# liamhebert/MultiModalDiscussionTransformer

Measured on AMD Instinct MI355X. Metric: discussion-tree comments/sec fwd+bwd, higher is better.
Workload: dtype bf16; 1 GPU; mDT-base (BERT-base + ViT-B/16 split 6+6, 6 executed graph layers, D768 H12 nb4 L100), 32 bushy 64-comment trees per GPU, 25% image comments, random-init weights, dropout 0.4/0.3/0.3 (run_train.sh:37), token lengths U{8..100} zero-padded to 100 (SURVEY.md §8d; mean 54.3 valid tokens), text side ragged: padded token positions are not computed (identical logits / gradients), last fusion layer comput; trees_per_gpu=32, parallelism=dp1, frozen_initial_encoders=False

## Files before the change

### multimodaldiscussiontransformer_amd/csrc/gemm.hip

```cpp
#include <stdlib.h>

#include <algorithm>
#include <type_traits>
#include <vector>

#include "common.hpp"
#include "gemm_tiles.hpp"
#include "gemm_epilogue.hpp"

namespace mdt {

template <typename TIn, typename TOut, bool TA, bool TB>
__global__ __launch_bounds__(256) void gemm_generic_kernel(GemmParams p) {
  constexpr int BM = 64, BN = 64, BK = 16, LD = 68;
  __shared__ float As[BK][LD];
  __shared__ float Bs[BK][LD];
  const int tid = threadIdx.x, lane = tid & 63, wave = tid >> 6;
  const int wr = wave >> 1, wc = wave & 1;
  const int64_t m0 = (int64_t)blockIdx.y * BM, n0 = (int64_t)blockIdx.x * BN;
  const int64_t kbeg = (int64_t)blockIdx.z * p.k_chunk;
  const int64_t kend = (kbeg + p.k_chunk < p.K) ? kbeg + p.k_chunk : p.K;
  const TIn* A = (const TIn*)p.A;
  const TIn* B = (const TIn*)p.B;
  f32x4 acc[2][2];
// ... 894 lines not shown
  }
  __shared__ float red[4][64 * VN];
#pragma unroll
  for (int e = 0; e < VN; ++e) red[wave][lane * VN + e] = acc[e];
  __syncthreads();
  for (int i = threadIdx.x; i < 64 * VN; i += 256) {
    const int64_t col = (int64_t)blockIdx.x * 64 * VN + i;
    if (col < N) atomicAdd(out + col, red[0][i] + red[1][i] + red[2][i] + red[3][i]);
  }
}

template <typename T>
__global__ __launch_bounds__(256) void dropout_kernel(int64_t rows, int D, const T* x, int64_t ldx, T* y, int64_t ldy, DropCfg d) {
  const int lane = threadIdx.x & 63;
  for (int64_t r = (int64_t)blockIdx.x * 4 + (threadIdx.x >> 6); r < rows; r += (int64_t)gridDim.x * 4)
    for (int c = lane; c < D; c += 64)
      y[r * ldy + c] = from_f32<T>(to_f32(x[r * ldx + c]) * drop_scale(d, (uint64_t)r * D + c));
}
template <typename T, int VN>
__global__ __launch_bounds__(256) void dropout_vec_kernel(int64_t rows, int D, const T* x, int64_t ldx, T* y, int64_t ldy, DropCfg d) {
  typedef __attribute__((ext_vector_type(VN))) T vec;
  const int lane = threadIdx.x & 63;
  for (int64_t r = (int64_t)blockIdx.x * 4 + (threadIdx.x >> 6); r < rows; r += (int64_t)gridDim.x * 4)
    for (int c = lane * VN; c < D; c += 64 * VN) {
      const vec v = *(const vec*)(x + r * ldx + c);
      vec o;
#pragma unroll
      for (int e = 0; e < VN; e += 2) {
        float s0, s1;
        drop_scale2(d, (uint64_t)r * D + c + e, s0, s1);
        o[e] = from_f32<T>(to_f32((T)v[e]) * s0);
        o[e + 1] = from_f32<T>(to_f32((T)v[e + 1]) * s1);
      }
      *(vec*)(y + r * ldy + c) = o;
    }
}
__global__ void dropout_mask_kernel(int64_t n, DropCfg d, uint8_t* mask) {
  for (int64_t i = (int64_t)blockIdx.x * blockDim.x + threadIdx.x; i < n; i += (int64_t)gridDim.x * blockDim.x)
    mask[i] = drop_scale(d, (uint64_t)i) != 0.f;
}

template <typename TS, typename TD>
__global__ void cast_kernel(int64_t n, const TS* s, TD* d) {
  for (int64_t i = (int64_t)blockIdx.x * blockDim.x + threadIdx.x; i < n; i += (int64_t)gridDim.x * blockDim.x)
    d[i] = from_f32<TD>(to_f32(s[i]));
}

template <typename TS, typename TD>
__global__ __launch_bounds__(256) void transpose_kernel(int64_t rows, int64_t cols, const TS* s, int64_t lds_, TD* d,
                                                        int64_t ldd) {
  __shared__ float tile[32][33];
  const int64_t r0 = (int64_t)blockIdx.y * 32, c0 = (int64_t)blockIdx.x * 32;
  const int tx = threadIdx.x & 31, ty = threadIdx.x >> 5;
  for (int i = ty; i < 32; i += 8)
    if (r0 + i < rows && c0 + tx < cols) tile[i][tx] = to_f32(s[(r0 + i) * lds_ + c0 + tx]);
  __syncthreads();
  for (int i = ty; i < 32; i += 8)
    if (c0 + i < cols && r0 + tx < rows) d[(c0 + i) * ldd + r0 + tx] = from_f32<TD>(tile[tx][i]);
}

static void report_stamps(unsigned long long* dev, size_t nwg, const GemmParams& p) {
  std::vector<unsigned long long> h(nwg * 4);
  if (hipDeviceSynchronize() != hipSuccess || hipMemcpy(h.data(), dev, nwg * 32, hipMemcpyDeviceToHost) != hipSuccess) { (void)hipGetLastError(); return; }
  std::vector<double> cyc, clk;
  unsigned long long t0 = ~0ull, t1 = 0;
  for (size_t i = 0; i < nwg; ++i) {
    if (h[4 * i + 2] == 0 || h[4 * i + 1] == 0) continue;
    cyc.push_back((double)h[4 * i] / (double)h[4 * i + 2]);
    clk.push_back((double)h[4 * i] / (double)h[4 * i + 1] * 100.0);
    t0 = std::min(t0, h[4 * i + 3]);
    t1 = std::max(t1, h[4 * i + 3] + h[4 * i + 1]);
  }
  if (cyc.empty()) return;
  std::sort(cyc.begin(), cyc.end());
  std::sort(clk.begin(), clk.end());
  fprintf(stderr, "[mdt gemm stamp] M=%lld N=%lld K=%lld wgs=%zu  cycles/k-tile median %.0f (p10 %.0f p90 %.0f)  clock median %.0f MHz  span %.1f us\n",
          (long long)p.M, (long long)p.N, (long long)p.K, nwg, cyc[cyc.size() / 2], cyc[cyc.size() / 10], cyc[cyc.size() * 9 / 10],
          clk[clk.size() / 2], (double)(t1 - t0) / 100.0);
  std::vector<unsigned long long> st(256);
  if (hipMemcpy(st.data(), dev + nwg * 4, 256 * 8, hipMemcpyDeviceToHost) == hipSuccess && st[0]) {
    fprintf(stderr, "[mdt gemm steps]");
    for (int i = 1; i < 256 && st[i]; ++i) fprintf(stderr, " %llu", st[i] - st[i - 1]);
    fprintf(stderr, "\n");
  } else (void)hipGetLastError();
}

static int num_cus() {
  const int n = device_cus() & ~7;
  return n < 8 ? 8 : n;
}

static int* g_tile_queues = nullptr;
static int g_tile_queue_sets = 0;

static int xcd_group_n(int tiles_m, int tiles_n, double b_panel, int n_cus) {
  if (tiles_n % 2 == 0 && b_panel * tiles_n > 3.5e6 && b_panel * (tiles_n / 2) <= 2.5e6 && (double)tiles_m * tiles_n >= 4.0 * n_cus)
    return tiles_n / 2;
  return tiles_n;
}

struct GemmPlan {
  GemmRoute route;
  int tiles_m, tiles_n, split_k, group_n;
  int64_t k_chunk;
  dim3 grid;
  bool strip_asum;
};

static GemmPlan plan_gemm(const GemmParams& p, int dtype, int out_dtype, int ta, int tb, int n_cus) {
  const Switches& sw = switches();
  const int64_t M = p.M, N = p.N, K = p.K;
  const int epi = p.epilogue;
  bool fast = dtype == MDT_BF16 && K > 0 && (ta ? M % T_BM == 0 : K % T_BK == 0) && (tb ? N % T_BN == 0 : K % T_BK == 0) &&
              N % T_BN == 0 && p.lda % 8 == 0 && p.ldb % 8 == 0 && ((uintptr_t)p.A | (uintptr_t)p.B) % 16 == 0 &&
              p.lda * 2 * 128 < (1ll << 31) && p.ldb * 2 * 128 < (1ll << 31);
  const int ov = out_dtype == MDT_F32 ? 4 : 8;
  if (!(epi & MDT_EPI_ATOMIC) && (p.ldc % ov || ((uintptr_t)p.C & 15))) fast = false;
  if ((epi & MDT_EPI_BIAS) && ((uintptr_t)p.bias & 15)) fast = false;
  if ((epi & MDT_EPI_RESIDUAL) && (p.ldr % 8 || ((uintptr_t)p.residual & 15))) fast = false;
  if (p.aux && (p.ldaux % 8 || ((uintptr_t)p.aux & 15))) fast = false;
  const int64_t chunk = ((K + p.split_k - 1) / p.split_k + T_BK - 1) / T_BK * T_BK;
  if (fast && (ta || tb) && chunk * (ta ? p.lda : p.ldb) * 2 >= (1ll << 32)) fast = false;
  const int split = fast ? (int)((K + chunk - 1) / chunk) : 1;

  const bool m256 = ta ? M % 256 == 0 : true;
  const int tm256 = (int)((M + 255) / 256), tn256 = (int)(N / 256);
  const bool pp = fast && m256 && N % 256 == 0;
  const int nhs = 2 * (int)((K + T_BK - 1) / T_BK);
  auto persist = [&](int min_steps) {
    return pp && out_dtype == MDT_BF16 && split == 1 && nhs >= min_steps && tm256 * tn256 > n_cus;
  };
  const bool queue = sw.gemm_dynamic && g_tile_queues;
  auto ok = [&](GemmRoute r) {
    switch (r) {
      case GemmRoute::generic: return true;
      case GemmRoute::tile128: return fast;
      case GemmRoute::tile256x128: return fast && m256;
      case GemmRoute::pp256: return pp;
      case GemmRoute::pp256p: return persist(4);
      case GemmRoute::w4p:
        return persist(16) && nhs >= W4_NEXPL + 2 && !queue && !(epi & (1 << 24));
      case GemmRoute::w4s:
        return pp && out_dtype == MDT_F32 && !sw.gemm_stamp && (epi & MDT_EPI_ATOMIC) &&
               !(epi & ((1 << 20) - 1) & ~(MDT_EPI_ATOMIC | MDT_EPI_ASUM)) && chunk >= 256 && K - (int64_t)(split - 1) * chunk >= 256;
      default: return false;
    }
  };
  GemmRoute r;
  const int64_t t256 = (int64_t)tm256 * (N / 128) * split;
  if (!fast) r = GemmRoute::generic;
  else if (pp && t256 / 2 >= 200) {
    const int e = epi & ((1 << 22) - 1);
    const bool light = e == 0 || e == MDT_EPI_BIAS || e == MDT_EPI_RESIDUAL || e == (MDT_EPI_BIAS | MDT_EPI_RESIDUAL | MDT_EPI_DROPOUT) ||
                       e == (MDT_EPI_MULAUX | MDT_EPI_COLSUM);
    if (persist(16)) r = ok(GemmRoute::w4p) && !ta && light ? GemmRoute::w4p : GemmRoute::pp256p;
    else r = ok(GemmRoute::w4s) ? GemmRoute::w4s : GemmRoute::pp256;
  } else if (m256 && t256 >= 256) r = GemmRoute::tile256x128;
  else r = GemmRoute::tile128;
  if (sw.gemm_route != GemmRoute::none && ok(sw.gemm_route)) r = sw.gemm_route;

  GemmPlan pl{};
  pl.route = r;
  pl.group_n = 1 << 30;
  pl.strip_asum = r != GemmRoute::pp256 && r != GemmRoute::w4s;
  if (r == GemmRoute::generic) {
    const int64_t c16 = ((K + p.split_k - 1) / p.split_k + 15) / 16 * 16;
    pl.k_chunk = c16 < 16 ? 16 : c16;
    pl.split_k = K > 0 ? (int)((K + pl.k_chunk - 1) / pl.k_chunk) : 1;
    pl.grid = dim3((unsigned)((N + 63) / 64), (unsigned)((M + 63) / 64), (unsigned)pl.split_k);
    return pl;
  }
  pl.k_chunk = chunk;
  pl.split_k = split;
  pl.tiles_m = r == GemmRoute::tile128 ? (int)((M + T_BM - 1) / T_BM) : tm256;
  pl.tiles_n = r == GemmRoute::tile128 || r == GemmRoute::tile256x128 ? (int)(N / T_BN) : tn256;
  pl.grid = dim3((unsigned)(pl.tiles_m * pl.tiles_n), 1, (unsigned)split);
  if (r == GemmRoute::tile128 || r == GemmRoute::tile256x128) return pl;
  pl.group_n = split > 1 ? (pl.tiles_n > pl.tiles_m ? 1 : pl.tiles_n) : xcd_group_n(pl.tiles_m, pl.tiles_n, 256.0 * (double)chunk * 2.0, n_cus);
  if (r == GemmRoute::pp256p || r == GemmRoute::w4p) pl.grid.x = (unsigned)n_cus;
  return pl;
}

constexpr int E_BIAS = MDT_EPI_BIAS, E_DENSE = MDT_EPI_BIAS | MDT_EPI_RESIDUAL | MDT_EPI_DROPOUT,
              E_FC1 = MDT_EPI_BIAS | MDT_EPI_GELU | MDT_EPI_AUX_GRAD , E_RES = MDT_EPI_RESIDUAL,
              E_DFC2 = MDT_EPI_MULAUX | MDT_EPI_COLSUM;
template <int E> using EpiK = std::integral_constant<int, E>;
template <bool A_KM, bool B_KM, class F>
static int with_epilogue(const GemmParams& p, F&& f) {
  const int e = p.epilogue & ((1 << 22) - 1);
  if constexpr (!A_KM && !B_KM) {
    if (e == E_BIAS) return f(EpiK<E_BIAS>{});
    if (e == E_DENSE) return f(EpiK<E_DENSE>{});
    if (e == E_FC1 && p.aux) return f(EpiK<E_FC1>{});
  }
  if constexpr (!A_KM) {
    if (e == 0) return f(EpiK<0>{});
    if (e == E_RES) return f(EpiK<E_RES>{});
    if (e == E_DFC2) return f(EpiK<E_DFC2>{});
  }
  return f(EpiK<-1>{});
}

template <class F>
static int with_layout(int ta, int tb, F&& f) {
  using T = std::true_type;
  using N = std::false_type;
  if (!ta && !tb) return f(N{}, N{});
  if (!ta) return f(N{}, T{});
  if (!tb) return f(T{}, N{});
  return f(T{}, T{});
}

template <typename TIn, typename TOut>
static int launch_generic(hipStream_t st, const GemmParams& p, dim3 grid, int ta, int tb) {
  return with_layout(ta, tb, [&](auto a_t, auto b_t) {
    return launch_route<gemm_generic_kernel<TIn, TOut, decltype(a_t)::value, decltype(b_t)::value>>("generic", grid, 256, 0, st, p);
  });
}

template <typename TOut>
static int launch_gemm(hipStream_t st, const GemmParams& p, GemmRoute r, dim3 grid, int ta, int tb) {
  const size_t pp_lds = (size_t)pp_nb(4) * PP_STAGE;
  const char* name = route_name(r);
  return with_layout(ta, tb, [&](auto a_km, auto b_km) -> int {
    constexpr bool A = decltype(a_km)::value, B = decltype(b_km)::value;
    switch (r) {
      case GemmRoute::tile128: return launch_route<gemm_bf16_tile128<TOut, A, B>>(name, grid, 256, 4 * T_TILE_BYTES, st, p);
      case GemmRoute::tile256x128:
        return launch_route<gemm_bf16_tile256<TOut, A, B, 128, 4, 2, 3>>(name, grid, 512, (size_t)3 * (256 + 128) * 128, st, p);
      case GemmRoute::pp256: return launch_route<gemm_bf16_pp256<TOut, A, B, 4>>(name, grid, 512, pp_lds, st, p);
      case GemmRoute::w4p:
        return with_epilogue<A, B>(p, [&](auto ek) {
          return launch_route<gemm_bf16_w4p<A, B, decltype(ek)::value>>(name, grid, 256, (size_t)5 * PP_STAGE, st, p);
        });
      case GemmRoute::pp256p:
        return with_epilogue<A, B>(p, [&](auto ek) {
          constexpr int EPK = decltype(ek)::value;
          if (!(p.epilogue & (1 << 24))) return launch_route<gemm_bf16_pp256p<A, B, 4, EPK>>(name, grid, 512, pp_lds, st, p);
          constexpr int EJ = (!B && (EPK == E_FC1 || EPK == E_DENSE)) || (B && EPK == E_DFC2) ? EPK : -1;
          return launch_route<gemm_bf16_pp256p<A, B, 4, EJ, 0, true>>(name, grid, 512, pp_lds, st, p);
        });
      default: set_error("mdt_gemm: route %s has no launch here", name); return MDT_ERR_ARG;
    }
  });
}

template <int F8>
static int launch_pp256p_f8(hipStream_t st, const GemmParams& p) {
  const int nvt = p.tiles_m * p.tiles_n;
  const dim3 grid((unsigned)(nvt < num_cus() ? nvt : num_cus()), 1, 1);
  const size_t lds = (size_t)pp_nb(4) * PP_STAGE;
  const int e = p.epilogue;
#define LF8(E_) return launch_route<gemm_bf16_pp256p<false, false, 4, E_, F8>>("f8_pp256p", grid, 512, lds, st, p)
  if constexpr (F8 == 1) {
    if (e == E_BIAS) LF8(E_BIAS);
    if (e == E_DENSE) LF8(E_DENSE);
    if (e == E_FC1 && p.aux) LF8(E_FC1);
  } else {
    if (e == 0) LF8(0);
    if (e == E_RES) LF8(E_RES);
    if (e == E_DFC2) LF8(E_DFC2);
  }
  LF8(-1);
#undef LF8
}

}

using namespace mdt;

extern "C" int mdt_gemm(void* stream, int dtype, int out_dtype, int trans_a, int trans_b, int64_t M, int64_t N,
                        int64_t K, const void* A, int64_t lda, const void* B, int64_t ldb, void* C, int64_t ldc,
                        int epilogue, float alpha, const void* bias, const void* residual, int64_t ldr, void* aux,
                        int64_t ldaux, int split_k, float drop_p, uint64_t drop_seed, float* colsum) {
  MDT_CHECK_ARG(dtype == MDT_F32 || dtype == MDT_BF16, "mdt_gemm: bad dtype %d", dtype);
  MDT_CHECK_ARG(out_dtype == MDT_F32 || out_dtype == MDT_BF16, "mdt_gemm: bad out_dtype %d", out_dtype);
  MDT_CHECK_ARG(M >= 0 && N >= 0 && K >= 0, "mdt_gemm: negative shape");
  if (M == 0 || N == 0) return MDT_OK;
  MDT_CHECK_ARG(A && B && C, "mdt_gemm: null operand");
  MDT_CHECK_ARG(!(epilogue & MDT_EPI_BIAS) || bias, "mdt_gemm: MDT_EPI_BIAS without bias");
  MDT_CHECK_ARG(!(epilogue & MDT_EPI_RESIDUAL) || residual, "mdt_gemm: MDT_EPI_RESIDUAL without residual");
  MDT_CHECK_ARG(!(epilogue & (MDT_EPI_DGELU | MDT_EPI_MULAUX)) || aux, "mdt_gemm: MDT_EPI_DGELU / MDT_EPI_MULAUX without aux");
  MDT_CHECK_ARG(!(epilogue & MDT_EPI_AUX_GRAD) || (epilogue & MDT_EPI_GELU), "mdt_gemm: MDT_EPI_AUX_GRAD needs MDT_EPI_GELU");
  MDT_CHECK_ARG(!(epilogue & MDT_EPI_ATOMIC) || out_dtype == MDT_F32, "mdt_gemm: MDT_EPI_ATOMIC needs fp32 C");
  MDT_CHECK_ARG(dtype == MDT_BF16 || out_dtype == MDT_F32, "mdt_gemm: fp32 inputs need fp32 output");
  if (split_k < 1) split_k = 1;
  MDT_CHECK_ARG(split_k == 1 || (epilogue & MDT_EPI_ATOMIC), "mdt_gemm: split_k > 1 needs MDT_EPI_ATOMIC");
  MDT_CHECK_ARG(!(epilogue & MDT_EPI_DROPOUT) || (drop_p >= 0.f && drop_p < 1.f), "mdt_gemm: dropout p=%f out of [0,1)", drop_p);
  MDT_CHECK_ARG(split_k == 1 || !(epilogue & (MDT_EPI_BIAS | MDT_EPI_GELU | MDT_EPI_RESIDUAL | MDT_EPI_DGELU | MDT_EPI_DROPOUT | MDT_EPI_MULAUX)),
                "mdt_gemm: split_k > 1 supports only the plain accumulate epilogue");
  hipStream_t st = (hipStream_t)stream;
  GemmParams p;
  p.M = M; p.N = N; p.K = K; p.A = A; p.lda = lda; p.B = B; p.ldb = ldb; p.C = C; p.ldc = ldc;
  p.epilogue = epilogue; p.alpha = alpha; p.bias = bias; p.residual = residual; p.ldr = ldr;
  p.aux = aux; p.ldaux = ldaux; p.split_k = split_k;
  MDT_CHECK_ARG(!(epilogue & MDT_EPI_DROPOUT) || M * N < DROP_MAX_ELEMS, "mdt_gemm: dropout site of %lld elements (limit 2^33)", (long long)(M * N));
  p.drop = make_drop((epilogue & MDT_EPI_DROPOUT) ? drop_p : 0.f, drop_seed);
  p.colsum = colsum;
  p.stamps = nullptr;
  p.tile_queue = nullptr;
  p.alpha_dev = p.alpha_dev2 = nullptr;
  p.epilogue |= switches().gemm_diag << 20;
  MDT_CHECK_ARG(!(epilogue & MDT_EPI_COLSUM) || (colsum && split_k == 1), "mdt_gemm: MDT_EPI_COLSUM needs a colsum buffer and split_k == 1");
  MDT_CHECK_ARG(!(epilogue & MDT_EPI_ASUM) || (colsum && trans_a && (epilogue & MDT_EPI_ATOMIC) && !(epilogue & MDT_EPI_COLSUM) && dtype == MDT_BF16 && out_dtype == MDT_F32),
                "mdt_gemm: MDT_EPI_ASUM needs bf16 operands, an fp32 C, trans_a = 1, MDT_EPI_ATOMIC, a colsum buffer and no MDT_EPI_COLSUM");
  const GemmPlan pl = plan_gemm(p, dtype, out_dtype, trans_a, trans_b, num_cus());
  p.k_chunk = pl.k_chunk; p.split_k = pl.split_k; p.tiles_m = pl.tiles_m; p.tiles_n = pl.tiles_n; p.group_n = pl.group_n;
  if (pl.strip_asum && (p.epilogue & MDT_EPI_ASUM)) {
    p.epilogue &= ~MDT_EPI_ASUM;
    if (int e = mdt_colsum(stream, dtype, K, M, A, lda, colsum, nullptr)) return e;
  }
  switch (pl.route) {
    case GemmRoute::generic:
      if (dtype == MDT_F32) return launch_generic<float, float>(st, p, pl.grid, trans_a, trans_b);
      return out_dtype == MDT_F32 ? launch_generic<bf16_t, float>(st, p, pl.grid, trans_a, trans_b)
                                  : launch_generic<bf16_t, bf16_t>(st, p, pl.grid, trans_a, trans_b);
    case GemmRoute::w4s: return launch_w4s(st, p, pl.grid, trans_a, trans_b);
    case GemmRoute::pp256p:
      if (switches().gemm_dynamic && g_tile_queues) {
        static unsigned turn = 0;
        p.tile_queue = g_tile_queues + 16 * (turn++ % (unsigned)g_tile_queue_sets);
      }
      [[fallthrough]];
    case GemmRoute::pp256:
      if (switches().gemm_stamp) {
        const size_t bytes = (size_t)pl.grid.x * pl.grid.z * 32 + 256 * 8;
        if (hipMalloc(&p.stamps, bytes) != hipSuccess) { (void)hipGetLastError(); p.stamps = nullptr; }
        else (void)hipMemsetAsync(p.stamps, 0, bytes, st);
      }
      break;
    default: break;
  }
  const int e = out_dtype == MDT_F32 ? launch_gemm<float>(st, p, pl.route, pl.grid, trans_a, trans_b)
                                     : launch_gemm<bf16_t>(st, p, pl.route, pl.grid, trans_a, trans_b);
  if (p.stamps) {
    if (e == MDT_OK) report_stamps(p.stamps, (size_t)pl.grid.x * pl.grid.z, p);
    (void)hipFree(p.stamps);
  }
  return e;
}

extern "C" size_t mdt_gemm_tile_queue_bytes(void) { return (size_t)512 * 16 * sizeof(int); }

extern "C" int mdt_gemm_set_tile_queue(void* zeroed_device_buffer, size_t bytes) {
  if (zeroed_device_buffer == nullptr) { g_tile_queues = nullptr; g_tile_queue_sets = 0; return MDT_OK; }
  MDT_CHECK_ARG(bytes >= 16 * sizeof(int) && ((uintptr_t)zeroed_device_buffer & 3) == 0, "mdt_gemm_set_tile_queue: buffer too small / unaligned");
  g_tile_queues = (int*)zeroed_device_buffer;
  g_tile_queue_sets = (int)(bytes / (16 * sizeof(int)));
  return MDT_OK;
}

extern "C" int mdt_gemm_fp8(void* stream, int a_format, int64_t M, int64_t N, int64_t K, const void* A, int64_t lda,
                            const void* B, int64_t ldb, void* C, int64_t ldc, int epilogue, const float* inv_scale_a,
                            const float* inv_scale_b, const void* bias, const void* residual, int64_t ldr, void* aux,
                            int64_t ldaux, float drop_p, uint64_t drop_seed, float* colsum) {
  return mdt_gemm_fp8_q8(stream, a_format, M, N, K, A, lda, B, ldb, C, ldc, epilogue, inv_scale_a, inv_scale_b, bias, residual, ldr,
                         aux, ldaux, drop_p, drop_seed, colsum, nullptr, 0, 0, nullptr, nullptr);
}

extern "C" int mdt_gemm_fp8_q8(void* stream, int a_format, int64_t M, int64_t N, int64_t K, const void* A, int64_t lda,
                               const void* B, int64_t ldb, void* C, int64_t ldc, int epilogue, const float* inv_scale_a,
                               const float* inv_scale_b, const void* bias, const void* residual, int64_t ldr, void* aux,
                               int64_t ldaux, float drop_p, uint64_t drop_seed, float* colsum, void* q8_out, int64_t ld_q8,
                               int q8_format, const float* q8_scale, float* q8_amax) {
  MDT_CHECK_ARG(a_format == 0 || a_format == 1, "mdt_gemm_fp8: a_format %d (0 = e4m3, 1 = e5m2)", a_format);
  MDT_CHECK_ARG(M >= 0 && N >= 0 && K >= 0, "mdt_gemm_fp8: negative shape");
  if (M == 0 || N == 0) return MDT_OK;
  MDT_CHECK_ARG(A && B && C && inv_scale_a && inv_scale_b, "mdt_gemm_fp8: null operand / scale");
  MDT_CHECK_ARG(!(epilogue & MDT_EPI_BIAS) || bias, "mdt_gemm_fp8: MDT_EPI_BIAS without bias");
  MDT_CHECK_ARG(!(epilogue & MDT_EPI_RESIDUAL) || residual, "mdt_gemm_fp8: MDT_EPI_RESIDUAL without residual");
  MDT_CHECK_ARG(!(epilogue & (MDT_EPI_DGELU | MDT_EPI_MULAUX)) || aux, "mdt_gemm_fp8: MDT_EPI_DGELU / MDT_EPI_MULAUX without aux");
  MDT_CHECK_ARG(!(epilogue & MDT_EPI_AUX_GRAD) || (epilogue & MDT_EPI_GELU), "mdt_gemm_fp8: MDT_EPI_AUX_GRAD needs MDT_EPI_GELU");
  MDT_CHECK_ARG(!(epilogue & (MDT_EPI_ATOMIC | MDT_EPI_ACCUM)), "mdt_gemm_fp8: bf16 store epilogues only");
  MDT_CHECK_ARG(!(epilogue & MDT_EPI_COLSUM) || colsum, "mdt_gemm_fp8: MDT_EPI_COLSUM needs a colsum buffer");
  MDT_CHECK_ARG(!(epilogue & MDT_EPI_DROPOUT) || (drop_p >= 0.f && drop_p < 1.f && M * N < DROP_MAX_ELEMS), "mdt_gemm_fp8: bad dropout site");
  const bool ok = N % 256 == 0 && K % 64 == 0 && K >= 256 && lda % 16 == 0 && ldb % 16 == 0 && (((uintptr_t)A | (uintptr_t)B) % 16 == 0) &&
                  ldc % 8 == 0 && ((uintptr_t)C & 15) == 0 && (!(epilogue & MDT_EPI_BIAS) || ((uintptr_t)bias & 15) == 0) &&
                  (!(epilogue & MDT_EPI_RESIDUAL) || (ldr % 8 == 0 && ((uintptr_t)residual & 15) == 0)) &&
                  (!aux || (ldaux % 8 == 0 && ((uintptr_t)aux & 15) == 0)) && lda * 256 < (1ll << 31) && ldb * 256 < (1ll << 31);
  if (!ok) MDT_UNSUPPORTED("mdt_gemm_fp8: shape M=%lld N=%lld K=%lld (needs N %% 256 == 0, K %% 64 == 0, K >= 256, 16-byte rows)",
                           (long long)M, (long long)N, (long long)K);
  GemmParams p;
  p.M = M; p.N = N; p.K = K; p.A = A; p.lda = lda; p.B = B; p.ldb = ldb; p.C = C; p.ldc = ldc;
  p.epilogue = epilogue; p.alpha = 1.0f; p.alpha_dev = inv_scale_a; p.alpha_dev2 = inv_scale_b;
  p.bias = bias; p.residual = residual; p.ldr = ldr; p.aux = aux; p.ldaux = ldaux; p.split_k = 1; p.k_chunk = K;
// ... 100 lines not shown
```

### multimodaldiscussiontransformer_amd/engine.py

```python
from __future__ import annotations

import os

import contextlib
import threading
import weakref
from dataclasses import dataclass
from typing import Callable, List, Optional, Sequence

import torch

from . import fp8 as F8
from . import ops


class _StreamState(threading.local):
    side_active = False


_SS = _StreamState()
_SIDE_STREAMS = {}


def side_stream(device) -> "torch.cuda.Stream":
    key = torch.device(device).index if torch.device(device).index is not None else torch.cuda.current_device()
    if key not in _SIDE_STREAMS:
        _SIDE_STREAMS[key] = torch.cuda.Stream(device=key)
    return _SIDE_STREAMS[key]


class Var:
    __slots__ = ("data", "grad", "needs_grad", "side")

    def __init__(self, data: torch.Tensor, needs_grad: bool = True):
        self.data = data
        self.grad: Optional[torch.Tensor] = None
        self.needs_grad = needs_grad
        self.side = _SS.side_active

    @property
    def rows(self):
        return self.data.shape[0]


class Tape:
    def __init__(self, use_main_grad: bool = False, on_params_ready: Optional[Callable] = None, inference: bool = False):
        self.ops: List[Callable[[], None]] = []
        self.inference = inference
        self.use_main_grad = use_main_grad
        self.tmp_grads = {}
        self.on_params_ready = on_params_ready
        self._seed_base = None
        self._seed_ctr = 0
        self.side: Optional[torch.cuda.Stream] = None
        self._main: Optional[torch.cuda.Stream] = None

    def enable_side(self, device):
        if self.side is None:
            self.side = side_stream(device)

    def fork(self):
        if self.side is None:
            return
        self.side.wait_stream(torch.cuda.current_stream())
        self.record(lambda: torch.cuda.current_stream().wait_stream(self.side))

    def join(self):
        if self.side is None:
            return
        torch.cuda.current_stream().wait_stream(self.side)
        self.record(lambda: self.side.wait_stream(torch.cuda.current_stream()))

    def _enter_side(self):
        self._main = torch.cuda.current_stream()
        torch.cuda.set_stream(self.side)
        _SS.side_active = True

    def _leave_side(self):
        if _SS.side_active:
            torch.cuda.set_stream(self._main)
            _SS.side_active = False

    @contextlib.contextmanager
    def on_side(self):
        if self.side is None:
            yield
            return
        self.record(self._leave_side)
        self._enter_side()
        try:
            yield
        finally:
            self._leave_side()
            self.record(self._enter_side)

    def _crossing(self, v: "Var", t: torch.Tensor):
        if self.side is not None and v.side != _SS.side_active:
            t.record_stream(self.side if v.side else self._main)

    def next_seed(self) -> int:
        if self._seed_base is None:
            self._seed_base = int(torch.randint(0, 2 ** 62, (1,)).item())
        self._seed_ctr += 1
        return (self._seed_base + 0x9E3779B97F4A7C15 * self._seed_ctr) & 0x7FFFFFFFFFFFFFFF

    def record(self, bwd: Callable[[], None]):
        if not self.inference:
            self.ops.append(bwd)

    def pgrad(self, p: torch.nn.Parameter) -> Optional[torch.Tensor]:
        if p is None or not p.requires_grad:
            return None
        if self.use_main_grad:
            g = getattr(p, "main_grad", None)
            if g is None:
                raise RuntimeError("use_main_grad=True but a trainable parameter has no .main_grad buffer")
            return g
        g = self.tmp_grads.get(id(p))
        if g is None:
            g = torch.zeros(p.shape, dtype=torch.float32, device=p.device)
            self.tmp_grads[id(p)] = g
        return g

    def grad_buf(self, v: Var) -> torch.Tensor:
        if v.grad is None:
            if self.side is not None and v.side and not _SS.side_active:
                with torch.cuda.stream(self.side):
                    v.grad = torch.zeros_like(v.data)
                torch.cuda.current_stream().wait_stream(self.side)
            else:
                v.grad = torch.zeros_like(v.data)
                self._crossing(v, v.grad)
        return v.grad

    def add_grad(self, v: Var, g: torch.Tensor):
        if not v.needs_grad:
            return
        if v.grad is None:
            v.grad = g
            self._crossing(v, g)
        else:
            ops.row_axpby(v.grad, v.grad.shape[0], a=g, accumulate=True)

    def backward(self):
        try:
            while self.ops:
                self.ops.pop()()
        finally:
            self._leave_side()
        self.ops = []
        self.sync_streams()
        if F8.ACTIVE is not None:
            F8.ACTIVE.end_of_step()

    def sync_streams(self):
        if self.side is not None:
            torch.cuda.current_stream().wait_stream(self.side)


@dataclass
class BlockParams:
    qkv_w: torch.nn.Parameter
    qkv_b: torch.nn.Parameter
    o_w: torch.nn.Parameter
    o_b: torch.nn.Parameter
    ln1_w: torch.nn.Parameter
    ln1_b: torch.nn.Parameter
    fc1_w: torch.nn.Parameter
    fc1_b: torch.nn.Parameter
    fc2_w: torch.nn.Parameter
    fc2_b: torch.nn.Parameter
    ln2_w: torch.nn.Parameter
    ln2_b: torch.nn.Parameter

    def all(self):
        return [self.qkv_w, self.qkv_b, self.o_w, self.o_b, self.ln1_w, self.ln1_b, self.fc1_w, self.fc1_b,
                self.fc2_w, self.fc2_b, self.ln2_w, self.ln2_b]


@dataclass
class AttnSpec:
    nseq: int
    S: int
    H: int
    seq_stride: Optional[int] = None
    pos_stride: int = 1
    scale: Optional[float] = None
    key_mask: Optional[torch.Tensor] = None
    dense_bias: Optional[torch.Tensor] = None
    dense_bias_var: Optional[Var] = None
    attn_bias: Optional[torch.Tensor] = None
    spatial_pos: Optional[torch.Tensor] = None
    sp_table: Optional[torch.nn.Parameter] = None
    virt: Optional[torch.nn.Parameter] = None
    key_pad: Optional[torch.Tensor] = None
    seq_offsets: Optional[torch.Tensor] = None
    q_limit: int = 0
    bins: Optional[list] = None

    def kwargs(self):
        return dict(seq_stride=self.seq_stride, pos_stride=self.pos_stride, scale=self.scale, key_mask=self.key_mask,
                    seq_offsets=self.seq_offsets, q_limit=self.q_limit, bins=self.bins,
                    dense_bias=self.dense_bias, attn_bias=self.attn_bias, spatial_pos=self.spatial_pos,
                    sp_table=None if self.sp_table is None else self.sp_table.data,
                    virt=None if self.virt is None else self.virt.data.view(-1), key_pad=self.key_pad)


def _split_k(n_out: int, k_out: int, red: int) -> int:
    tiles = ((n_out + 127) // 128) * ((k_out + 127) // 128)
    s = max(1, 1024 // max(1, tiles))
    return int(max(1, min(s, red // 1024 if red >= 1024 else 1)))


_WGRAD_ASUM = os.environ.get("MDT_WGRAD_ASUM", "1") != "0"


def wgrad(tape: Tape, dy: torch.Tensor, x: torch.Tensor, w: torch.nn.Parameter, b: Optional[torch.nn.Parameter]):
    gw = tape.pgrad(w)
    gb = tape.pgrad(b) if b is not None else None
    if gw is not None:
        ride = gb is not None and dy.dtype == torch.bfloat16 and _WGRAD_ASUM
        ops.gemm(dy, x, trans_a=True, trans_b=True, out=gw.view(dy.shape[1], x.shape[1]), epilogue=ops.EPI_ATOMIC,
                 split_k=_split_k(dy.shape[1], x.shape[1], dy.shape[0]), asum=gb.view(-1) if ride else None)
        if ride:
            return
    if gb is not None:
        ops.colsum(dy, out=gb.view(-1))


_LN_BIAS_RIDE = os.environ.get("MDT_LN_BIAS_RIDE", "1") != "0"


EMBED_LN_FUSED = os.environ.get("MDT_EMBED_LN_FUSED", "1") != "0"
PATCH_K_PAD = os.environ.get("MDT_PATCH_K_PAD", "1") != "0"
PATCH_EMBED_FUSED = os.environ.get("MDT_PATCH_EMBED_FUSED", "1") != "0"
WEIGHT_EPOCH = 0


def weights_changed():
    global WEIGHT_EPOCH
    WEIGHT_EPOCH += 1


_KP_CACHE: dict = {}


def _k_padded(w: torch.nn.Parameter, wmat: torch.Tensor, kp: int) -> torch.Tensor:
    key = (id(w), kp)
    ver = (w._version, WEIGHT_EPOCH, w.data_ptr())
    hit = _KP_CACHE.get(key)
    if hit is not None and hit[0]() is w and hit[1] == ver:
        return hit[2]
    wp = torch.zeros(wmat.shape[0], kp, dtype=wmat.dtype, device=wmat.device)
    wp[:, :wmat.shape[1]].copy_(wmat)
    _KP_CACHE[key] = (weakref.ref(w), ver, wp)
    return wp


def dgrad(dy: torch.Tensor, w: torch.nn.Parameter, **kw) -> torch.Tensor:
    return ops.gemm(dy, w.data, trans_b=True, **kw)


def linear(f8, x: torch.Tensor, w: torch.nn.Parameter, tag: str, *, grad=False, x8=None, q8_site=None, q8_grad=False, **kw):
    r = None if f8 is None else f8.linear(x, w, (tag, id(w)), transposed_weight=grad, grad=grad, x8=x8, q8_site=q8_site,
                                          q8_grad=q8_grad, **kw)
    if r is None:
        return (dgrad(x, w, **kw) if grad else ops.gemm(x, w.data, **kw)), None
    return r if q8_site is not None else (r, None)


def dyd_rides(g: torch.Tensor) -> bool:
    return _LN_BIAS_RIDE and g.dtype == torch.bfloat16 and g.shape[0] >= 8192


def _ln_bwd(tape, dy, x, w, b, mean, rstd, add=None):
    return ops.layernorm_bwd(dy, x, w.data, mean, rstd, add=add, dgamma=tape.pgrad(w), dbeta=tape.pgrad(b))


def _ln_bwd_dense(tape, dy, x, w, b, mean, rstd, bias_param, p_drop, seed, add=None):
    gb = tape.pgrad(bias_param) if bias_param is not None else None
    return ops.layernorm_bwd(dy, x, w.data, mean, rstd, add=add, dgamma=tape.pgrad(w), dbeta=tape.pgrad(b),
                             drop_p=p_drop, drop_seed=seed, colsum=None if gb is None else gb.view(-1),
                             want_dropped=True)


def transformer_block(tape: Tape, x: Var, P: BlockParams, spec: AttnSpec, *, pre_ln: bool, eps: float,
                      p_hidden: float = 0.0, p_attn: float = 0.0, p_act: float = 0.0, keep_rows=None) -> Var:
    xd = x.data
    s_attn, s_o, s_act, s_f2 = (tape.next_seed() for _ in range(4))
    kw = dict(spec.kwargs(), drop_p=p_attn, drop_seed=s_attn)
    R = None if keep_rows is None else int(keep_rows.numel())
    f8 = F8.ACTIVE

    def gather(src):
        if keep_rows is None:
            return src
        out_ = torch.empty(R, src.shape[1], dtype=src.dtype, device=src.device)
        ops.row_axpby(out_, R, a=src, ai=keep_rows)
        return out_

    def spread(g_):
        if keep_rows is None:
            return g_
        full = torch.zeros(xd.shape[0], g_.shape[1], dtype=g_.dtype, device=g_.device)
        ops.row_axpby(full, R, di=keep_rows, a=g_)
        return full

    def ln8(x_, lw, lb, w_, tag):
        slot = None if (f8 is None or x_.dtype != torch.bfloat16) else f8.producer_slot(x_.shape[0], w_, (tag, id(w_)))
        if slot is None:
            return (*ops.layernorm_fwd(x_, lw.data, lb.data, eps), None)
        return (*ops.layernorm_fwd(x_, lw.data, lb.data, eps, q8=slot[:4]), (slot[0], slot[4]))

    def attn_fwd(src, src8):
        qkv_, _ = linear(f8, src, P.qkv_w, "qkv", x8=src8, bias=P.qkv_b.data)
        ctx_full_, lse_ = ops.attention_fwd(qkv_, spec.nseq, spec.S, spec.H, **kw)
        ctx_, xk = gather(ctx_full_), gather(xd)
        return qkv_, ctx_full_, lse_, ctx_, ops.gemm(ctx_, P.o_w.data, bias=P.o_b.data, residual=xk, drop_p=p_hidden, drop_seed=s_o)

    def ffn_fwd(src, src8, res):
        u_ = torch.empty(src.shape[0], P.fc1_w.shape[0], dtype=src.dtype, device=src.device)
        h_, h8 = linear(f8, src, P.fc1_w, "fc1", x8=src8, q8_site=("fc2", id(P.fc2_w)), bias=P.fc1_b.data, aux=u_,
                        epilogue=ops.EPI_GELU | ops.EPI_AUX_GRAD, drop_p=p_act, drop_seed=s_act)
        return u_, h_, linear(f8, h_, P.fc2_w, "fc2", x8=h8, bias=P.fc2_b.data, residual=res, drop_p=p_hidden, drop_seed=s_f2)[0]

    if not pre_ln:
        a_in = xd
        qkv, ctx_full, lse, ctx, t = attn_fwd(a_in, None)
        f_in, m1, r1, f_in8 = ln8(t, P.ln1_w, P.ln1_b, P.fc1_w, "fc1")
        u, h, y = ffn_fwd(f_in, f_in8, f_in)
        out, m2, r2 = ops.layernorm_fwd(y, P.ln2_w.data, P.ln2_b.data, eps)
    else:
        a_in, m1, r1, a_in8 = ln8(xd, P.ln1_w, P.ln1_b, P.qkv_w, "qkv")
        qkv, ctx_full, lse, ctx, t = attn_fwd(a_in, a_in8)
        f_in, m2, r2, f_in8 = ln8(t, P.ln2_w, P.ln2_b, P.fc1_w, "fc1")
        u, h, out = ffn_fwd(f_in, f_in8, t)
    o = Var(out)

    def ffn_bwd(gd, fc2_b, dres):
        wgrad(tape, gd, h, P.fc2_w, fc2_b)
        gb1 = tape.pgrad(P.fc1_b)
        du, du8 = linear(f8, gd, P.fc2_w, "d_fc2", grad=True, q8_site=("d_fc1", id(P.fc1_w)), q8_grad=True, aux=u,
                         epilogue=ops.EPI_MULAUX, colsum=None if gb1 is None else gb1.view(-1))
        wgrad(tape, du, f_in, P.fc1_w, None)
        return linear(f8, du, P.fc1_w, "d_fc1", grad=True, x8=du8, residual=dres)[0]

    def attn_bwd(dtd, o_b, want_dx, dres=None):
        wgrad(tape, dtd, ctx, P.o_w, o_b)
        dctx = ops.gemm(dtd, P.o_w.data, trans_b=True)
        dqkv = _attention_bwd(tape, spec, kw, dctx, qkv, ctx_full, lse, spread)
        wgrad(tape, dqkv, a_in, P.qkv_w, P.qkv_b)
        return dgrad(dqkv, P.qkv_w, residual=None if dres is None else spread(dres)) if want_dx else None

    def bwd():
        g = o.grad
        o.grad = None
        if g is None:
            return
        ride = _WGRAD_ASUM and dyd_rides(g)
        if not pre_ln:
            dy, dyd = _ln_bwd_dense(tape, g, y, P.ln2_w, P.ln2_b, m2, r2, None if ride else P.fc2_b, p_hidden, s_f2)
            df = ffn_bwd(dyd, P.fc2_b if ride else None, dy)
            dt_, dtd = _ln_bwd_dense(tape, df, t, P.ln1_w, P.ln1_b, m1, r1, None if ride else P.o_b, p_hidden, s_o)
            dx = attn_bwd(dtd, P.o_b if ride else None, x.needs_grad, dt_)
            if x.needs_grad:
                tape.add_grad(x, dx)
        else:
            gd = ops.dropout(g, p_hidden, s_f2) if p_hidden > 0 else g
            df = ffn_bwd(gd, P.fc2_b, None)
            dt_, dtd = _ln_bwd_dense(tape, df, t, P.ln2_w, P.ln2_b, m2, r2, None if ride else P.o_b, p_hidden, s_o, add=g)
            da = attn_bwd(dtd, P.o_b if ride else None, True)
            if x.needs_grad:
                tape.add_grad(x, _ln_bwd(tape, da, xd, P.ln1_w, P.ln1_b, m1, r1, add=spread(dt_)))
            else:
                _ln_bwd(tape, da, xd, P.ln1_w, P.ln1_b, m1, r1)
        if tape.on_params_ready:
            tape.on_params_ready(P.all())

    tape.record(bwd)
    return o


def _attention_bwd(tape: Tape, spec: AttnSpec, kw: dict, dctx, qkv, ctx, lse, spread=lambda g: g):
    extra = {}
    if spec.sp_table is not None:
        extra = dict(d_sp_table=tape.pgrad(spec.sp_table),
                     d_virt=None if tape.pgrad(spec.virt) is None else tape.pgrad(spec.virt).view(-1))
    want_dense = spec.dense_bias_var is not None and spec.dense_bias_var.needs_grad
    dqkv, dbias = ops.attention_bwd(spread(dctx), qkv, ctx, lse, spec.nseq, spec.S, spec.H, **kw, want_dense_dbias=want_dense,
                                    **extra)
    if want_dense:
        tape.add_grad(spec.dense_bias_var, dbias)
    return dqkv


def attention_layer(tape: Tape, x: Var, qkv_w, qkv_b, o_w, o_b, spec: AttnSpec, p_attn: float = 0.0, stash: Optional[dict] = None) -> Var:
    xd = x.data
    kw = dict(spec.kwargs(), drop_p=p_attn, drop_seed=tape.next_seed())
    qkv = ops.gemm(xd, qkv_w.data, bias=None if qkv_b is None else qkv_b.data)
    ctx, lse = ops.attention_fwd(qkv, spec.nseq, spec.S, spec.H, **kw)
    if stash is not None:
        stash.update(qkv=qkv, lse=lse, kw=spec.kwargs())
    out = ops.gemm(ctx, o_w.data, bias=None if o_b is None else o_b.data)
    o = Var(out)

    def bwd():
        g = o.grad
        o.grad = None
        if g is None:
            return
        wgrad(tape, g, ctx, o_w, o_b)
        dqkv = _attention_bwd(tape, spec, kw, ops.gemm(g, o_w.data, trans_b=True), qkv, ctx, lse)
        wgrad(tape, dqkv, xd, qkv_w, qkv_b)
        if x.needs_grad:
            tape.add_grad(x, ops.gemm(dqkv, qkv_w.data, trans_b=True))

    tape.record(bwd)
    return o


def layernorm(tape: Tape, x: Var, w, b, eps: float) -> Var:
    y, mean, rstd = ops.layernorm_fwd(x.data, w.data, b.data, eps)
    o = Var(y)

    def bwd():
        g = o.grad
        o.grad = None
        if g is None:
            return
        dx = _ln_bwd(tape, g, x.data, w, b, mean, rstd)
        tape.add_grad(x, dx)

    tape.record(bwd)
    return o


def dropout(tape: Tape, x: Var, p: float) -> Var:
    if p <= 0.0:
        return x
    seed = tape.next_seed()
    o = Var(ops.dropout(x.data, p, seed))

    def bwd():
        g = o.grad
        o.grad = None
        if g is None:
            return
        tape.add_grad(x, ops.dropout(g, p, seed))

    tape.record(bwd)
    return o


def bert_embeddings(tape: Tape, ids, types, word, pos, typ) -> Var:
    M, Lq = ids.shape
    D = word.shape[1]
    out = torch.empty(M * Lq, D, dtype=word.dtype, device=word.device)
    ops.bert_embed_sum(ids, types, word.data, pos.data, typ.data, out, out_seq_stride=Lq, out_off=0)
    o = Var(out)

    def bwd():
        g = o.grad
        o.grad = None
        if g is None:
            return
        gw, gp, gt = tape.pgrad(word), tape.pgrad(pos), tape.pgrad(typ)
        if gw is not None:
            ops.row_scatter_add(gw, ids.view(-1), g, M * Lq)
        if gp is not None:
            ops.colsum(g.view(M, Lq * D), out=gp[:Lq].view(-1))
        if gt is not None:
            assert typ.shape[0] == 2, "token-type gradient is implemented for type_vocab_size == 2"
            tot = ops.colsum(g)
            one = ops.colsum(g, row_weight=types.view(-1))
            ops.row_axpby(gt, 1, d_off=1, a=one.view(1, D), accumulate=True)
            ops.row_axpby(gt, 1, d_off=0, a=tot.view(1, D), b=one.view(1, D), beta=-1.0, accumulate=True)

    tape.record(bwd)
    return o


def _embed_rows_grads(tape: Tape, g, rows, ids, types, pos_ids, word, pos, typ):
    gw, gp, gt = tape.pgrad(word), tape.pgrad(pos), tape.pgrad(typ)
    D = word.shape[1]
    if gw is not None:
        ops.row_scatter_add(gw, ids, g, rows)
    if gp is not None:
        ops.row_scatter_add(gp, pos_ids, g, rows)
    if gt is not None:
        assert typ.shape[0] == 2, "token-type gradient is implemented for type_vocab_size == 2"
        tot = ops.colsum(g)
        one = ops.colsum(g, row_weight=types)
        ops.row_axpby(gt, 1, d_off=1, a=one.view(1, D), accumulate=True)
        ops.row_axpby(gt, 1, d_off=0, a=tot.view(1, D), b=one.view(1, D), beta=-1.0, accumulate=True)


def bert_embeddings_rows(tape: Tape, ids, types, pos_ids, word, pos, typ) -> Var:
    rows = ids.numel()
    D = word.shape[1]
    out = torch.empty(rows, D, dtype=word.dtype, device=word.device)
    ops.bert_embed_rows(ids, types, pos_ids, word.data, pos.data, typ.data, out)
    o = Var(out)

    def bwd():
        g = o.grad
        o.grad = None
        if g is None:
            return
        _embed_rows_grads(tape, g, rows, ids, types, pos_ids, word, pos, typ)

    tape.record(bwd)
    return o


def bert_embeddings_ln_rows(tape: Tape, ids, types, pos_ids, word, pos, typ, w, b, eps: float) -> Var:
    rows = ids.numel()
    y, mean, rstd, xs = ops.bert_embed_ln_rows(ids, types, pos_ids, word.data, pos.data, typ.data, w.data, b.data, eps,
                                               keep_sum=not tape.inference)
    o = Var(y)

    def bwd():
        g = o.grad
        o.grad = None
        if g is None:
            return
        dx = _ln_bwd(tape, g, xs, w, b, mean, rstd)
        _embed_rows_grads(tape, dx, rows, ids, types, pos_ids, word, pos, typ)

    tape.record(bwd)
    return o


# ... 280 lines not shown
```

Before: 16220 comments/s.

## Ride fc1 bias grad on wgrad and hand dropout grad down between pre-LN layers

The fc1 bias gradient is now accumulated in the fc1 weight-gradient GEMM through its row-sum path, so the d_fc2 GEMM no longer needs a colsum epilogue. A MULAUX-only epilogue is added to the w4p persistent kernel so that GEMM can stay on the fast route. Between consecutive pre-LN layers, the LayerNorm backward of the upper layer also writes the dropout-masked gradient that the lower layer's output dropout needs. This removes a separate dropout pass over the gradient. In exchange it adds cross-layer bookkeeping on Var (drop_site, grad_dropped) that must be invalidated correctly when gradients accumulate.

```diff
diff --git a/multimodaldiscussiontransformer_amd/csrc/gemm.hip b/multimodaldiscussiontransformer_amd/csrc/gemm.hip
--- a/multimodaldiscussiontransformer_amd/csrc/gemm.hip
+++ b/multimodaldiscussiontransformer_amd/csrc/gemm.hip
@@ -1070,7 +1070,7 @@
   else if (pp && t256 / 2 >= 200) {
     const int e = epi & ((1 << 22) - 1);
     const bool light = e == 0 || e == MDT_EPI_BIAS || e == MDT_EPI_RESIDUAL || e == (MDT_EPI_BIAS | MDT_EPI_RESIDUAL | MDT_EPI_DROPOUT) ||
-                       e == (MDT_EPI_MULAUX | MDT_EPI_COLSUM);
+                       e == (MDT_EPI_MULAUX | MDT_EPI_COLSUM) || e == MDT_EPI_MULAUX;
     if (persist(16)) r = ok(GemmRoute::w4p) && !ta && light ? GemmRoute::w4p : GemmRoute::pp256p;
     else r = ok(GemmRoute::w4s) ? GemmRoute::w4s : GemmRoute::pp256;
   } else if (m256 && t256 >= 256) r = GemmRoute::tile256x128;
@@ -1101,9 +1101,10 @@
 
 constexpr int E_BIAS = MDT_EPI_BIAS, E_DENSE = MDT_EPI_BIAS | MDT_EPI_RESIDUAL | MDT_EPI_DROPOUT,
               E_FC1 = MDT_EPI_BIAS | MDT_EPI_GELU | MDT_EPI_AUX_GRAD , E_RES = MDT_EPI_RESIDUAL,
-              E_DFC2 = MDT_EPI_MULAUX | MDT_EPI_COLSUM;
+              E_DFC2 = MDT_EPI_MULAUX | MDT_EPI_COLSUM,
+              E_DFC2M = MDT_EPI_MULAUX ;
 template <int E> using EpiK = std::integral_constant<int, E>;
-template <bool A_KM, bool B_KM, class F>
+template <bool A_KM, bool B_KM, bool W4 = false, class F>
 static int with_epilogue(const GemmParams& p, F&& f) {
   const int e = p.epilogue & ((1 << 22) - 1);
   if constexpr (!A_KM && !B_KM) {
@@ -1115,6 +1116,9 @@
     if (e == 0) return f(EpiK<0>{});
     if (e == E_RES) return f(EpiK<E_RES>{});
     if (e == E_DFC2) return f(EpiK<E_DFC2>{});
+    if constexpr (W4) {
+      if (e == E_DFC2M) return f(EpiK<E_DFC2M>{});
+    }
   }
   return f(EpiK<-1>{});
 }
@@ -1148,7 +1152,7 @@
         return launch_route<gemm_bf16_tile256<TOut, A, B, 128, 4, 2, 3>>(name, grid, 512, (size_t)3 * (256 + 128) * 128, st, p);
       case GemmRoute::pp256: return launch_route<gemm_bf16_pp256<TOut, A, B, 4>>(name, grid, 512, pp_lds, st, p);
       case GemmRoute::w4p:
-        return with_epilogue<A, B>(p, [&](auto ek) {
+        return with_epilogue<A, B, true>(p, [&](auto ek) {
           return launch_route<gemm_bf16_w4p<A, B, decltype(ek)::value>>(name, grid, 256, (size_t)5 * PP_STAGE, st, p);
         });
       case GemmRoute::pp256p:
diff --git a/multimodaldiscussiontransformer_amd/engine.py b/multimodaldiscussiontransformer_amd/engine.py
--- a/multimodaldiscussiontransformer_amd/engine.py
+++ b/multimodaldiscussiontransformer_amd/engine.py
@@ -30,13 +30,15 @@
 
 
 class Var:
-    __slots__ = ("data", "grad", "needs_grad", "side")
+    __slots__ = ("data", "grad", "needs_grad", "side", "drop_site", "grad_dropped")
 
     def __init__(self, data: torch.Tensor, needs_grad: bool = True):
         self.data = data
         self.grad: Optional[torch.Tensor] = None
         self.needs_grad = needs_grad
         self.side = _SS.side_active
+        self.drop_site = None
+        self.grad_dropped = None
 
     @property
     def rows(self):
@@ -131,11 +133,13 @@
             else:
                 v.grad = torch.zeros_like(v.data)
                 self._crossing(v, v.grad)
+        v.grad_dropped = None
         return v.grad
 
     def add_grad(self, v: Var, g: torch.Tensor):
         if not v.needs_grad:
             return
+        v.grad_dropped = None
         if v.grad is None:
             v.grad = g
             self._crossing(v, g)
@@ -229,6 +233,8 @@
 
 
 _LN_BIAS_RIDE = os.environ.get("MDT_LN_BIAS_RIDE", "1") != "0"
+_FC1_BIAS_RIDE = os.environ.get("MDT_FC1_BIAS_RIDE", "1") != "0"
+_DROP_HANDDOWN = os.environ.get("MDT_DROP_HANDDOWN", "1") != "0"
 
 
 EMBED_LN_FUSED = os.environ.get("MDT_EMBED_LN_FUSED", "1") != "0"
@@ -291,6 +297,8 @@
     kw = dict(spec.kwargs(), drop_p=p_attn, drop_seed=s_attn)
     R = None if keep_rows is None else int(keep_rows.numel())
     f8 = F8.ACTIVE
+    hand = x.drop_site if (pre_ln and keep_rows is None and not tape.inference and x.drop_site is not None
+                           and x.drop_site[2] == len(tape.ops)) else None
 
     def gather(src):
         if keep_rows is None:
@@ -340,9 +348,11 @@
     def ffn_bwd(gd, fc2_b, dres):
         wgrad(tape, gd, h, P.fc2_w, fc2_b)
         gb1 = tape.pgrad(P.fc1_b)
+        ride1 = (_FC1_BIAS_RIDE and _WGRAD_ASUM and f8 is None and gd.dtype == torch.bfloat16 and gd.shape[0] >= 8192 and
+                 tape.pgrad(P.fc1_w) is not None)
         du, du8 = linear(f8, gd, P.fc2_w, "d_fc2", grad=True, q8_site=("d_fc1", id(P.fc1_w)), q8_grad=True, aux=u,
-                         epilogue=ops.EPI_MULAUX, colsum=None if gb1 is None else gb1.view(-1))
-        wgrad(tape, du, f_in, P.fc1_w, None)
+                         epilogue=ops.EPI_MULAUX, colsum=None if gb1 is None or ride1 else gb1.view(-1))
+        wgrad(tape, du, f_in, P.fc1_w, P.fc1_b if ride1 else None)
         return linear(f8, du, P.fc1_w, "d_fc1", grad=True, x8=du8, residual=dres)[0]
 
     def attn_bwd(dtd, o_b, want_dx, dres=None):
@@ -366,11 +376,22 @@
             if x.needs_grad:
                 tape.add_grad(x, dx)
         else:
-            gd = ops.dropout(g, p_hidden, s_f2) if p_hidden > 0 else g
+            hd, o.grad_dropped = o.grad_dropped, None
+            if p_hidden <= 0:
+                gd = g
+            elif hd is not None and hd[0] is g:
+                gd = hd[1]
+            else:
+                gd = ops.dropout(g, p_hidden, s_f2)
             df = ffn_bwd(gd, P.fc2_b, None)
             dt_, dtd = _ln_bwd_dense(tape, df, t, P.ln2_w, P.ln2_b, m2, r2, None if ride else P.o_b, p_hidden, s_o, add=g)
             da = attn_bwd(dtd, P.o_b if ride else None, True)
-            if x.needs_grad:
+            if x.needs_grad and hand is not None and x.grad is None:
+                dx, dxd = ops.layernorm_bwd(da, xd, P.ln1_w.data, m1, r1, add=dt_, dgamma=tape.pgrad(P.ln1_w),
+                                            dbeta=tape.pgrad(P.ln1_b), drop_p=hand[0], drop_seed=hand[1], want_dropped=True)
+                tape.add_grad(x, dx)
+                x.grad_dropped = (dx, dxd)
+            elif x.needs_grad:
                 tape.add_grad(x, _ln_bwd(tape, da, xd, P.ln1_w, P.ln1_b, m1, r1, add=spread(dt_)))
             else:
                 _ln_bwd(tape, da, xd, P.ln1_w, P.ln1_b, m1, r1)
@@ -378,6 +399,8 @@
             tape.on_params_ready(P.all())
 
     tape.record(bwd)
+    if pre_ln and p_hidden > 0 and _DROP_HANDDOWN:
+        o.drop_site = (p_hidden, s_f2, len(tape.ops))
     return o
 
 
```

Result: no change. 16210 comments/s (-0.1%).
